# snowflakezzz/FAST-LIVO-noted

Measured on AMD Instinct MI355X. Metric: IEKF scan-to-map updates/sec (100k-pt scan, 1M-pt map), higher is better.
Workload: dtype f32+f64; 1 GPU; config2: 100k-pt scan vs 1M-pt map, max_iteration=4, 8 independent scans per GPU per step; scan_points=100000, map_points=1000000, parallelism=scan farm x1

## Files before the change

fast-livo-noted_amd/csrc/livo_capi.cpp:

```cpp
#include <hip/hip_runtime.h>

#include <algorithm>
#include <cmath>
#include <cstdio>
#include <cstdlib>
#include <cstring>
#include <new>
#include <chrono>
#include <thread>
#include <vector>

#include "carve.h"
#include "livo_internal.h"

using namespace livo;

namespace {

struct ScanBuf {
    bool used = false;
    int64_t n = 0;
    int32_t nblk = 0;
    float* pts = nullptr;
    NNRec* nn = nullptr;
// ... 138 lines not shown
    int32_t dvlog2 = 4;
    int64_t d_n = 0, dslot_cap = 0, dpts_cap = 0;
    int64_t rebases = 0;
    double rebase_frac = 0.125;
    float min_gh = 0.f;
    float max_gh = 0.f;
    float box_cell = 1.2f;
    float box_cell_max = 2.0f;
    float* gpts_alt = nullptr;
    int64_t gpts_alt_cap = 0;
    int64_t grid_ids = -1, cells = -1;
    float grid_gh = 0.f;
    bool merge = true;
    int64_t rebuilds_sorted = 0, rebuilds_merged = 0;
    int64_t wide_redos = 0;
    int64_t rebuilds_fused = 0;
    ScanCtx scan;
};

struct Staging {
    char* h = nullptr;
    char* d = nullptr;
    char* h_dev = nullptr;
    size_t cap = 0;
    void free() {
        if (d) (void)hipFree(d);
        if (h) (void)hipHostFree(h);
        h = d = h_dev = nullptr;
        cap = 0;
    }
    int ensure(size_t bytes) {
        if (bytes <= cap) return LIVO_OK;
        free();
        if (hipMalloc((void**)&d, bytes) != hipSuccess) {
            d = nullptr;
            return LIVO_E_OOM;
        }
        if (hipHostMalloc((void**)&h, bytes, hipHostMallocMapped | hipHostMallocCoherent) != hipSuccess) {
            h = nullptr;
            return LIVO_E_OOM;
        }
        if (hipHostGetDevicePointer((void**)&h_dev, h, 0) != hipSuccess) {
            (void)hipGetLastError();
            h_dev = nullptr;
        }
        cap = bytes;
        return LIVO_OK;
    }
};

struct BatchPlan {
    int model = 0;
    int32_t n = 0;
    bool fused = false;
    bool kcopy = false;
    bool wb = false;
    bool iv = false;
    bool lazy = false;
    int prof = 0;
    Staging* stage = nullptr;
    size_t stride = 0;
    int ngroups = 0;
    struct Group {
        int32_t first, count;
        int max_nblk;
        int64_t max_n, off;
        hipStream_t st;
    } g[kMaxGroups];
};

struct BatchLane {
    Staging stage[2];
    hipStream_t st[kMaxGroups] = {};
    hipEvent_t done[kMaxGroups] = {};
    bool busy = false;
    int32_t ticket = -1;
    int32_t n = 0;
    BatchPlan plan;
    std::vector<int32_t> ids;
};

constexpr int kPinRing = 16;

struct livo_ctx {
    int device = 0;
    hipStream_t stream = nullptr;
    hipStream_t xstream[kMaxGroups - 1] = {};
    hipEvent_t xjoin[kMaxGroups - 1] = {};
    int groups = 0;
    int leaf_size = kLeafSize;
    livo_params params{};
    MapNode* nodes = nullptr;
    int64_t map_points = 0;
    int64_t map_slots = 0;
    int32_t map_depth = 0;
    LeafNode* lnodes = nullptr;
    float* lpts = nullptr;
    int32_t leaf_depth = 0;
    int64_t leaf_bytes = 0;
    int knn_kind = 2;
// ... 37 lines not shown
    DevImage match_img;
    void* vm_buf = nullptr;
    size_t vm_bytes = 0;
    void* prim_tmp = nullptr;
    size_t prim_bytes = 0;
    std::vector<ScanBuf> scans;
    std::vector<ScanBuf> spare;
    void* up_tmp = nullptr;
    size_t up_tmp_bytes = 0;
    hipStream_t up_stream = nullptr;
    void* aup_tmp = nullptr;
    size_t aup_tmp_bytes = 0;
    void* aup_prim = nullptr;
    size_t aup_prim_bytes = 0;
    struct PinSlot {
        float* h = nullptr;
        size_t bytes = 0;
        hipEvent_t copied = nullptr;
        bool inflight = false;
    } pin[kPinRing];
    int pin_next = 0;
    hipStream_t cp_stream = nullptr;
    void* bsrc[2] = {nullptr, nullptr};
    size_t bsrc_bytes[2] = {0, 0};
    hipEvent_t bsrc_copied[2] = {nullptr, nullptr};
    hipEvent_t bsrc_free[2] = {nullptr, nullptr};
    bool bsrc_used[2] = {false, false};
    int bsrc_next = 0;
    IekfSlot* d_slots = nullptr;
    BatchLane lane[LIVO_MAX_INFLIGHT];
    int32_t lane_gen = 0;
    bool lane_serial = false;
    bool slot_wb = true;
    bool rec_compact = true;
    bool rec_lazy = true;
    bool eval_gen = false;
    int last_lane = -1;
    unsigned long long last_replays = 0;
    IekfSlot* h_slots = nullptr;
    HsJob* d_jobs = nullptr;
    HsJob* h_jobs = nullptr;
    unsigned* d_replay_count = nullptr;
    unsigned long long* d_replay_total = nullptr;
    unsigned long long* d_replay_list = nullptr;
    int64_t replay_cap = 0;
    unsigned* d_replay_count2 = nullptr;
    unsigned long long* d_replay_list2 = nullptr;
    void* scratch = nullptr;
    size_t scratch_bytes = 0;
    void* rec_tmp = nullptr;
    size_t rec_tmp_bytes = 0;
    int profiling = 0;
    hipEvent_t ev[kMaxGroups][3 * LIVO_MAX_EVALS + 2] = {};
    hipEvent_t b_start = nullptr, b_end[2] = {};
    int b_par = 0;
    bool b_prev = false;
    bool events_ready = false;
    livo_timings last{};
};

#define HIP_TRY(x)                                  \
    do {                                            \
        if ((x) != hipSuccess) return LIVO_E_HIP;   \
    } while (0)
#define RC_TRY(x)                  \
    do {                           \
// ... 1318 lines not shown
    livo_params def;
    livo_params_default(&def);
    if (p && !params_valid(p)) return LIVO_E_INVALID;
    int ndev = 0;
    if (hipGetDeviceCount(&ndev) != hipSuccess || ndev <= 0) return LIVO_E_HIP;
    if (device < 0 || device >= ndev) return LIVO_E_INVALID;
    livo_ctx* c = new (std::nothrow) livo_ctx();
    if (!c) return LIVO_E_OOM;
    c->device = device;
    c->params = p ? *p : def;
    if (const char* env = std::getenv("LIVO_STREAM_GROUPS")) {
        const int v = std::atoi(env);
        if (v >= 1 && v <= kMaxGroups) c->groups = v;
    }
    if (const char* env = std::getenv("LIVO_LEAF_SIZE")) {
        const int v = std::atoi(env);
        if (v >= 2 && v <= 256) c->leaf_size = v;
    }
    if (const char* env = std::getenv("LIVO_FUSED")) c->fused = std::atoi(env) != 0;
    if (const char* env = std::getenv("LIVO_KNN_KIND"))
        c->knn_kind = std::strcmp(env, "leaf") == 0 ? 0 : std::strcmp(env, "grid") == 0 ? 1 : 2;
    if (const char* env = std::getenv("LIVO_VRUNS")) c->vruns = std::atoi(env) != 0;
    if (const char* env = std::getenv("LIVO_BRUNS")) c->bruns = std::atoi(env) != 0;
    if (const char* env = std::getenv("LIVO_BR_HA")) {
        const float v = (float)std::atof(env);
        if (v > 0.2f && v < 20.f) c->br_ha = v;
    }
    if (const char* env = std::getenv("LIVO_BR_R")) {
        const float v = (float)std::atof(env);
        if (v > 0.5f && v < 20.f) c->br_r = v;
    }
    if (const char* env = std::getenv("LIVO_LANE_SERIAL")) c->lane_serial = std::atoi(env) != 0;
    if (const char* env = std::getenv("LIVO_SLOT_WB")) c->slot_wb = std::atoi(env) != 0;
    if (const char* env = std::getenv("LIVO_REC_COMPACT")) c->rec_compact = std::atoi(env) != 0;
    if (const char* env = std::getenv("LIVO_REC_LAZY")) c->rec_lazy = std::atoi(env) != 0;
    if (const char* env = std::getenv("LIVO_EVAL_GEN")) c->eval_gen = std::atoi(env) != 0;
    if (const char* env = std::getenv("LIVO_XCD_CHUNK")) c->xcd_chunk = std::max(0, std::atoi(env));
    if (const char* env = std::getenv("LIVO_GRID_PPC")) {
        const float v = (float)std::atof(env);
        if (v > 0.f) c->grid_ppc = v;
    }
    if (const char* env = std::getenv("LIVO_GRID_CELL")) {
        const float v = (float)std::atof(env);
        if (v > 0.f) c->grid_cell = v;
    }
    if (set_device(c) || hipStreamCreateWithFlags(&c->stream, hipStreamNonBlocking) != hipSuccess ||
        create_group_streams(c)) {
        delete c;
        return LIVO_E_HIP;
    }
    *out = c;
    return LIVO_OK;
}

int livo_ctx_destroy(livo_ctx* c) {
    if (!c) return LIVO_E_INVALID;
    (void)hipSetDevice(c->device);
    if (c->stream) (void)hipStreamSynchronize(c->stream);
    for (int k = 0; k < kMaxGroups - 1; k++)
        if (c->xstream[k]) (void)hipStreamSynchronize(c->xstream[k]);
    if (c->up_stream) (void)hipStreamSynchronize(c->up_stream);
    if (c->cp_stream) (void)hipStreamSynchronize(c->cp_stream);
    for (int k = 0; k < 2; k++) {
        if (c->bsrc[k]) (void)hipFree(c->bsrc[k]);
        if (c->bsrc_copied[k]) (void)hipEventDestroy(c->bsrc_copied[k]);
        if (c->bsrc_free[k]) (void)hipEventDestroy(c->bsrc_free[k]);
// ... 1257 lines not shown
    std::sort(sorted.begin(), sorted.end());
    if (std::adjacent_find(sorted.begin(), sorted.end()) != sorted.end()) return LIVO_E_INVALID;
    for (int l = 0; l < LIVO_MAX_INFLIGHT; l++)
        if (l != L && c->lane[l].busy)
            for (int32_t id : c->lane[l].ids)
                if (std::binary_search(sorted.begin(), sorted.end(), id)) return LIVO_E_INVALID;
    if (!batch_fused(c, model) && model != kModelIkfom && (L != 0 || !sync)) return LIVO_E_INVALID;
    return LIVO_OK;
}

static int64_t batch_plan(livo_ctx* c, int L, int32_t n, const int32_t* ids, int model, bool sync) {
    BatchLane& B = c->lane[L];
    BatchPlan& P = B.plan;
    P.model = model;
    P.n = n;
    P.fused = batch_fused(c, model);
    P.stage = &B.stage[model];
    P.stride = model == kModelIkfom ? sizeof(IekfSlot) : kLmStride;
    P.kcopy = !sync && P.stage->h_dev;
    P.wb = P.fused && P.stage->h_dev && c->slot_wb;
    P.iv = c->backend == LIVO_BACKEND_IVOX && model != kModelIkfom;
    P.prof = sync && L == 0 && c->events_ready ? c->profiling : 0;
    const int auto_groups = (P.fused || model == kModelIkfom) ? 4 : 2;
    P.ngroups = std::max(1, std::min<int>(c->groups > 0 ? c->groups : auto_groups, n));
    int64_t off = 0;
    for (int gi = 0; gi < P.ngroups; gi++) {
        BatchPlan::Group& G = P.g[gi];
        G.first = (int32_t)((int64_t)n * gi / P.ngroups);
        G.count = (int32_t)((int64_t)n * (gi + 1) / P.ngroups) - G.first;
        G.max_nblk = 1;
        G.max_n = 1;
        G.off = off;
        G.st = B.st[gi];
        for (int32_t b = G.first; b < G.first + G.count; b++) {
            const ScanBuf* s = get_scan_q(c, ids[b]);
            G.max_nblk = std::max(G.max_nblk, (int)s->nblk);
            G.max_n = std::max<int64_t>(G.max_n, s->n);
            off += s->n;
        }
    }
    return off;
}

static void batch_fill(livo_ctx* c, const BatchPlan& P, const int32_t* ids, const livo_state* states,
                       const livo_state* priors, const livo_ikfom_state* ik_states) {
    HsJob* const hjobs = reinterpret_cast<HsJob*>(P.stage->h + (size_t)P.n * P.stride);
    const int max_iter = c->params.max_iterations;
    for (int32_t b = 0; b < P.n; b++) {
        if (P.model == kModelIkfom) {
            init_slot_ik(hslot(P, b), ik_states[b], max_iter);
        } else {
            init_slot(hslot(P, b), states[b], priors ? priors[b] : states[b], max_iter, kSlotLmBytes);
        }
        fill_job(hjobs[b], *get_scan_q(c, ids[b]), dslot(P, b));
        if (P.wb) hjobs[b].host_slot = reinterpret_cast<uint4*>(P.stage->h_dev + (size_t)b * P.stride);
    }
}

static unsigned* lane_rcount(livo_ctx* c, int L) { return c->d_replay_count + (size_t)L * kMaxGroups; }

static int stage_group(livo_ctx* c, int L, const BatchPlan& P, int gi, const int32_t* ids, const BatchLane* prev) {
    static_assert(sizeof(HsJob) % 16 == 0 && sizeof(IekfSlot) % 16 == 0 && kLmStride % 16 == 0, "16-B word copies");
    const BatchPlan::Group& G = P.g[gi];
    const hipStream_t st = G.st;
    for (int32_t b = G.first; b < G.first + G.count; b++) {
        ScanBuf* s = get_scan_q(c, ids[b]);
        if (s->pending) HIP_TRY(hipStreamWaitEvent(st, s->ready, 0));
        if (P.model == kModelIkfom && s->n > 0) HIP_TRY(hipMemsetAsync(s->pstate, 0, (size_t)s->n, st));
        if (!P.fused) RC_TRY(ensure_nn_coords(c, s, st));
    }
    if (prev)
        for (int q = 0; q < prev->plan.ngroups; q++) HIP_TRY(hipStreamWaitEvent(st, prev->done[q], 0));
    const size_t s0 = (size_t)G.first * P.stride, sb = (size_t)G.count * P.stride;
    const size_t j0 = (size_t)P.n * P.stride + (size_t)G.first * sizeof(HsJob), jb = (size_t)G.count * sizeof(HsJob);
    if (P.kcopy) {
        RC_TRY(launch_copy_ranges(P.stage->h_dev, P.stage->d, s0, sb, j0, jb, st));
    } else {
        HIP_TRY(hipMemcpyAsync(P.stage->d + s0, P.stage->h + s0, sb, hipMemcpyHostToDevice, st));
        HIP_TRY(hipMemcpyAsync(P.stage->d + j0, P.stage->h + j0, jb, hipMemcpyHostToDevice, st));
    }
    if (!P.fused) HIP_TRY(hipMemsetAsync(lane_rcount(c, L) + gi, 0, sizeof(unsigned), st));
    if (P.iv) HIP_TRY(hipMemsetAsync(c->d_replay_count2 + gi, 0, sizeof(unsigned), st));
    HIP_TRY(prof_record(P, kProfAny, c->ev[gi][0], st));
    return LIVO_OK;
}

static void group_params(livo_ctx* c, int L, const BatchPlan& P, int gi, KnnParams& kp, HsParams& hp) {
    const BatchPlan::Group& G = P.g[gi];
    HsJob* const jobs = reinterpret_cast<HsJob*>(P.stage->d + (size_t)P.n * P.stride) + G.first;
    hp = make_hs_params(c);
    hp.jobs = jobs;
    kp = make_knn_params(c);
    kp.jobs = jobs;
    kp.replay_count = lane_rcount(c, L) + gi;
    kp.replay_list = c->d_replay_list + (size_t)L * c->replay_cap + G.off;
    kp.replay_count2 = P.iv ? c->d_replay_count2 + gi : nullptr;
    kp.replay_list2 = P.iv ? c->d_replay_list2 + G.off : nullptr;
    if (kp.iv.scratch) kp.iv.scratch += (int64_t)gi * c->iv.big_threads * c->iv.big_slice;
    hp.solve = P.model == kModelIkfom ? 0 : 1;
    hp.replay_count = kp.replay_count;
    hp.replay_count2 = kp.replay_count2;
}

static int queue_fused(livo_ctx* c, const BatchPlan& P, const int32_t* ids, const KnnParams* kp, const HsParams* hp) {
    for (int32_t b = 0; b < P.n; b++) {
        ScanBuf* s = get_scan_q(c, ids[b]);
        s->nn_lazy = false;
        if (kp[0].rec_compact) s->nn_compact = true;
    }
    const int evals = c->params.max_iterations + 1;
    for (int e = 0; e < evals; e++)
        for (int gi = 0; gi < P.ngroups; gi++) {
            const BatchPlan::Group& G = P.g[gi];
            if (e > 0) HIP_TRY(prof_record(P, kProfL2, c->ev[gi][e], G.st));
            RC_TRY(launch_iekf_eval(kp[gi], hp[gi], G.count, G.max_n, e == 0, G.st));
            if (e == 0) HIP_TRY(prof_record(P, kProfL1, c->ev[gi][1], G.st));
        }
    return LIVO_OK;
}

static int queue_unfused(livo_ctx* c, const BatchPlan& P, const KnnParams* kp, const HsParams* hp) {
    const int evals = c->params.max_iterations + 1;
    const bool ik = P.model == kModelIkfom;
    for (int e = 0; e < evals; e++)
        for (int gi = 0; gi < P.ngroups; gi++) {
            const BatchPlan::Group& G = P.g[gi];
            if (e > 0) HIP_TRY(prof_record(P, kProfL2, c->ev[gi][3 * e], G.st));
            RC_TRY(backend_knn(c, kp[gi], G.count, G.max_n, e > 0, G.st));
            HIP_TRY(prof_record(P, e == 0 ? kProfAny : kProfL2, c->ev[gi][3 * e + 1], G.st));
            RC_TRY(ik ? launch_hshare_ik(hp[gi], G.count, G.max_nblk, e == 0, G.st)
                      : launch_hshare(hp[gi], G.count, G.max_nblk, e == 0, G.st));
            if (ik) RC_TRY(launch_solve_ik(hp[gi], G.count, G.st));
        }
    return LIVO_OK;
}

static int finish_group(livo_ctx* c, BatchLane& B, const BatchPlan& P, int gi) {
    const BatchPlan::Group& G = P.g[gi];
    const int last_ev = P.fused ? c->params.max_iterations + 1 : 3 * LIVO_MAX_EVALS;
    HIP_TRY(prof_record(P, kProfL2, c->ev[gi][last_ev], G.st));
    if (P.wb) {
    } else if (P.kcopy) {
        RC_TRY(launch_copy_words(dslot(P, G.first), P.stage->h_dev + (size_t)G.first * P.stride, P.stride * G.count,
                                 G.st));
    } else {
        HIP_TRY(hipMemcpyAsync(&hslot(P, G.first), dslot(P, G.first), P.stride * G.count, hipMemcpyDeviceToHost, G.st));
    }
    HIP_TRY(hipEventRecord(B.done[gi], G.st));
// ... 1449 lines not shown
```

fast-livo-noted_amd/csrc/livo_internal.h:

```cpp
#pragma once
#include <math.h>
#include <stddef.h>
#include <stdint.h>

#include "cam_model.h"
#include "vmap_model.h"
#include "livo.h"
#include "stl_select.h"

#ifndef LIVO_PTS_PER_THREAD
#define LIVO_PTS_PER_THREAD 1
#endif

namespace livo {

constexpr int kRunPad = 8;

constexpr int kNN = LIVO_NUM_MATCH_POINTS;
constexpr int kDim = LIVO_DIM_STATE;
constexpr int kBlock = 256;
#ifndef LIVO_KNN_BLOCK
#define LIVO_KNN_BLOCK 128
#endif
constexpr int kKnnBlock = LIVO_KNN_BLOCK;
// ... 282 lines not shown
    int32_t rec_lazy;
    int32_t eval_gen;
};

struct SolveParams {
    IekfSlot* slots;
    const HsJob* jobs;
    unsigned* replay_count;
    int32_t mode;
};

struct HostMap {
    MapNode* nodes = nullptr;
    int64_t num_points = 0;
    int64_t num_slots = 0;
    int32_t depth = 0;
};
int build_host_map(const float* xyz, int64_t M, int64_t stride_bytes, HostMap* out);
void free_host_map(HostMap* m);

size_t knn_lds_bytes(int depth);
int launch_knn_pass(const KnnParams& p, int n_jobs, int64_t max_n, void* stream);
int launch_knn_leaf(const KnnParams& p, int n_jobs, int64_t max_n, bool seeded, void* stream);
int launch_knn_grid(const KnnParams& p, int n_jobs, int64_t max_n, bool seeded, bool tile, void* stream);
int launch_hshare(const HsParams& p, int n_jobs, int max_nblk, bool first, void* stream);
#ifndef LIVO_EVAL_BLOCK
#define LIVO_EVAL_BLOCK 256
#endif
constexpr int kEvalBlock = LIVO_EVAL_BLOCK;
enum EvalKind : int { kEvalRunsStatic = 0, kEvalGeneric = 1 };
#ifndef LIVO_EVAL_WAVES
#define LIVO_EVAL_WAVES 5
#endif
int launch_iekf_eval(const KnnParams& kp, const HsParams& hp, int n_jobs, int64_t max_n, bool first, void* stream);
int launch_solve_ik(const HsParams& p, int n_jobs, void* stream);
int launch_copy_words(const void* src, void* dst, size_t bytes, void* stream);
int launch_copy_ranges(const void* src, void* dst, size_t o0, size_t n0, size_t o1, size_t n1, void* stream);
int launch_hshare_ik(const HsParams& p, int n_jobs, int max_nblk, bool first, void* stream);
int launch_solve(const SolveParams& p, int n_jobs, void* stream);

int launch_ivox_clear(GridSlot* slots, int64_t table, void* stream);
int launch_ivox_insert(const IvoxParams& p, void* stream);
int launch_ivox_rollback(const IvoxParams& p, void* stream);
int launch_ivox_prepare(const IvoxParams& p, void* stream);
int launch_ivox_move(const IvoxParams& p, void* stream);
int launch_ivox_place(const IvoxParams& p, void* stream);
int launch_ivox_fix(const IvoxParams& p, void* stream);
int launch_ivox_rehash(const GridSlot* old_slots, const unsigned long long* old_t, int64_t old_table, GridSlot* slots,
                       unsigned long long* tlast, int log2, void* stream);
int launch_ivox_newfirst(const IvoxParams& p, uint32_t* out, unsigned long long* n, void* stream);
int launch_ivox_oldkeys(const IvoxParams& p, unsigned long long* keys, uint32_t* slot, unsigned long long* n,
                        void* stream);
int launch_ivox_untouched(const IvoxParams& p, const uint32_t* sorted_slot, int64_t n, uint32_t* flags, void* stream);
int launch_ivox_oldfirst(const IvoxParams& p, const uint32_t* sorted_slot, int64_t n, uint32_t* out, void* stream);
int launch_ivox_victims(const IvoxParams& p, const uint32_t* sorted_slot, const uint32_t* rank, int64_t n, int64_t ev,
                        uint32_t j_first, void* stream);
int launch_ivox_tcur_min(const IvoxParams& p, void* stream);
int launch_ivox_mark_min(const IvoxParams& p, void* stream);
int launch_ivox_drop(const IvoxParams& p, void* stream);
int launch_ivox_commit(const IvoxParams& p, void* stream);
int launch_ivox_knn(const KnnParams& p, int n_jobs, int64_t max_n, bool later, int64_t overflow_threads,
                    void* stream);
int prim_sort_pairs_u32(void* temp, size_t* temp_bytes, const uint32_t* keys_in, uint32_t* keys_out,
                        const uint32_t* vals_in, uint32_t* vals_out, int64_t n, int bits, void* stream);
int prim_exclusive_scan_u32(void* temp, size_t* temp_bytes, const uint32_t* in, uint32_t* out, int64_t n,
                            void* stream);
struct MapIncrParams {
// ... 347 lines not shown
```

fast-livo-noted_amd/csrc/livo_kernels.hip:

```cpp
#include <hip/hip_runtime.h>
#include <math.h>

#include <utility>

#include "livo_internal.h"
#include "device_common.h"
#include "device_linalg.h"

#if defined(LIVO_EVAL_PROF) && !defined(LIVO_TAIL_PROF)
#define LIVO_TAIL_PROF
#endif

namespace livo {

template <class T>
__device__ __forceinline__ const __attribute__((address_space(1))) T* gptr(const T* p) {
    return (const __attribute__((address_space(1))) T*)p;
}
template <class T>
__device__ __forceinline__ __attribute__((address_space(1))) T* gptr(T* p) {
    return (__attribute__((address_space(1))) T*)p;
}
constexpr double kMtkTol = 1e-11;
constexpr double kS2Len = 98090.0 / 10000.0;
// ... 2296 lines not shown
    bfly_stage<0x1B>(x, 4, (l & 2) == 0);
    bfly_stage<0xB1>(x, 2, (l & 1) == 0);
    const int base = ((l & 8) ? 16 : 0) + ((l & 4) ? 8 : 0) + ((l & 2) ? 4 : 0) + ((l & 1) ? 2 : 0);
    if (base < NU) R.red[(tid >> 4) * kRedCols + base] = x[0];
    if (base + 1 < NU) R.red[(tid >> 4) * kRedCols + base + 1] = x[1];
}

#ifdef LIVO_TAIL_PROF
__device__ unsigned long long g_tail_prof[3][8];
#define TAIL_MARK(k, t)                                                                                 \
    do {                                                                                               \
        if (pk >= 0 && threadIdx.x == 0) {                                                             \
            const unsigned long long now_ = __builtin_amdgcn_s_memtime();                             \
            atomicAdd(&g_tail_prof[pk][(k)], now_ - (t));                                              \
            (t) = now_;                                                                                \
        }                                                                                              \
    } while (0)
#else
#define TAIL_MARK(k, t) do { } while (0)
#endif
#ifndef LIVO_RED_INFLIGHT
#define LIVO_RED_INFLIGHT 32
#endif
constexpr int kRedInFlight = LIVO_RED_INFLIGHT;
__device__ __forceinline__ void hs_host_slot(const HsJob& job, const IekfSlot* slot, int t, int nt) {
    const unsigned long long* src = reinterpret_cast<const unsigned long long*>(slot);
    for (int w = t; w < (int)((kSlotWbBytes + 15) / 16); w += nt) {
        const unsigned long long lo = __hip_atomic_load(gptr(src + 2 * w), __ATOMIC_RELAXED, __HIP_MEMORY_SCOPE_AGENT);
        const unsigned long long hi = __hip_atomic_load(gptr(src + 2 * w + 1), __ATOMIC_RELAXED, __HIP_MEMORY_SCOPE_AGENT);
        job.host_slot[w] = make_uint4((unsigned)lo, (unsigned)(lo >> 32), (unsigned)hi, (unsigned)(hi >> 32));
    }
}

template <int NT, int NU, class Col>
__device__ __forceinline__ void hs_block_partial(const HsJob& job, const Col& col, unsigned blk, HsReduceLds& R) {
    const int tid = threadIdx.x;
    constexpr int NR = NT / 16;
    static_assert(NR <= kRedRows, "HsReduceLds row partials");
    constexpr int NRM = NR > 16 ? NR : 16;
    hs_row_sums_bfly<NU>(col, R, tid, std::make_integer_sequence<int, 32>{});
    __syncthreads();
    if (tid < NU) {
        double r[NRM];
#pragma unroll
        for (int w = 0; w < NRM; w++) r[w] = w < NR ? R.red[w * kRedCols + tid] : 0.0;
#pragma unroll
        for (int h = NRM / 2; h >= 1; h >>= 1)
#pragma unroll
            for (int w = 0; w < h; w++) r[w] = r[w] + r[w + h];
        const double v = r[0];
        __hip_atomic_store(gptr(job.partial + (size_t)blk * kRedCols + tid), v, __ATOMIC_RELAXED, __HIP_MEMORY_SCOPE_AGENT);
    }
}

template <int NT, int NU>
__device__ __forceinline__ void hs_scan_tail(const HsParams& P, const HsJob& job, IekfSlot* slot, int nblk,
                                             HsReduceLds& R, SolveLds& L, int pk
#ifdef LIVO_TAIL_PROF
                                             , unsigned long long tp
#endif
);

template <int NT, int NU = kRedUsed>
__device__ __forceinline__ bool hs_shard_level(const HsJob& job, IekfSlot* slot, int nblk, unsigned blk,
                                               HsReduceLds& R) {
    static_assert(NU == kRedUsed || NU == kRedUsed + 2, "h_share sums (+ search counts)");
    static_assert(NT / 32 <= kRedRows / 2, "R.fin holds one row per 32-thread group");
    const int tid = threadIdx.x;
    const int K = nblk < kRedShards ? nblk : kRedShards;
    const int sh = (int)(blk % (unsigned)K);
    const int cnt = (nblk - sh + K - 1) / K;
    unsigned* const sh_ticket = slot->sh_ticket + 32 * sh;
    if (tid < 64) {
        asm volatile("s_waitcnt vmcnt(0)" ::: "memory");
        if (tid == 0)
            R.last = __hip_atomic_fetch_add(gptr(sh_ticket), 1u, __ATOMIC_RELAXED, __HIP_MEMORY_SCOPE_AGENT) ==
                     (unsigned)cnt - 1u;
    }
    __syncthreads();
    if (!R.last) return false;
    if (cnt > 1) {
        constexpr int G = NT / 32;
        constexpr int kMaxPer = 8;
        const int c = tid & 31, g = tid >> 5;
        double acc = 0.0;
        if (c < NU) {
            const double* src = job.partial + c;
            for (int j0 = g; j0 < cnt; j0 += kMaxPer * G) {
                double v[kMaxPer];
#pragma unroll
                for (int k = 0; k < kMaxPer; k++) {
                    const int j = j0 + G * k;
                    v[k] = j < cnt ? ld_sc1(src + (size_t)(sh + K * j) * kRedCols) : 0.0;
                }
#pragma unroll
                for (int k = 0; k < kMaxPer; k++) acc += v[k];
            }
        }
        R.fin[g * kRedCols + c] = acc;
        __syncthreads();
        if (tid < NU) {
            constexpr int NG = G > 8 ? G : 8;
            double f[NG];
#pragma unroll
            for (int q = 0; q < NG; q++) f[q] = q < G ? R.fin[q * kRedCols + tid] : 0.0;
#pragma unroll
            for (int h = NG / 2; h >= 1; h >>= 1)
#pragma unroll
                for (int q = 0; q < h; q++) f[q] = f[2 * q] + f[2 * q + 1];
            st_sc1(job.partial + (size_t)sh * kRedCols + tid, f[0]);
        }
    }
    if (tid < 64) {
        if (tid == 0) st_sc1(sh_ticket, 0u);
        asm volatile("s_waitcnt vmcnt(0)" ::: "memory");
    }
    return true;
}

template <int NT, int NU = kRedUsed>
__device__ __forceinline__ void hs_ticket_tail(const HsParams& P, const HsJob& job, IekfSlot* slot, int nblk,
                                               unsigned blk, HsReduceLds& R, SolveLds& L, int pk = -1) {
    const int tid = threadIdx.x;
#ifdef LIVO_TAIL_PROF
    unsigned long long tp = __builtin_amdgcn_s_memtime();
    if (pk >= 0 && tid == 0) atomicAdd(&g_tail_prof[pk][0], 1ull);
#else
    (void)pk;
#endif
    if (!hs_shard_level<NT, NU>(job, slot, nblk, blk, R)) return;
    TAIL_MARK(1, tp);
    const int K = nblk < kRedShards ? nblk : kRedShards;
    if (tid == 0)
        R.last2 = __hip_atomic_fetch_add(gptr(&slot->hs_ticket), 1u, __ATOMIC_RELAXED, __HIP_MEMORY_SCOPE_AGENT) ==
                  (unsigned)K - 1u;
    __syncthreads();
    if (!R.last2) return;
#ifdef LIVO_TAIL_PROF
    hs_scan_tail<NT, NU>(P, job, slot, K, R, L, pk, tp);
#else
    hs_scan_tail<NT, NU>(P, job, slot, K, R, L, pk);
#endif
}

template <int NT, int NU>
__device__ __forceinline__ void hs_scan_tail(const HsParams& P, const HsJob& job, IekfSlot* slot, int nblk,
                                             HsReduceLds& R, SolveLds& L, int pk
#ifdef LIVO_TAIL_PROF
                                             , unsigned long long tp
#endif
) {
    const int tid = threadIdx.x;
    __builtin_amdgcn_s_setprio(3);
#ifdef LIVO_TAIL_PROF
    if (pk >= 0 && tid == 0) atomicAdd(&g_tail_prof[pk][5], 1ull);
#endif
    const bool solve = P.solve != 0;
    if (solve) solve_stage(slot, L, tid, NT);
    {
        constexpr int G = NT / 32;
        const int c = tid & 31, g = tid >> 5;
        double acc = 0.0;
        if (c < NU) {
            double* src = job.partial + c;
            for (int b0 = g; b0 < nblk; b0 += kRedInFlight * G) {
                double v[kRedInFlight];
#pragma unroll
                for (int k = 0; k < kRedInFlight; k++) {
                    const int b = b0 + G * k;
                    v[k] = b < nblk ? ld_sc1(src + (size_t)b * kRedCols) : 0.0;
                }
#pragma unroll
                for (int k = 0; k < kRedInFlight; k++) acc += v[k];
            }
        }
        R.fin[g * kRedCols + c] = acc;
    }
    __syncthreads();
    const bool wb = solve && job.host_slot != nullptr;
    if (tid >= 64) {
        if (solve && tid == 64) state_minus_d(L.pr, L.st, L.vec);
        if (solve) __syncthreads();
        if (wb) {
            __syncthreads();
            if (L.ctrl.stop) hs_host_slot(job, slot, tid, NT);
        }
        return;
    }
    TAIL_MARK(2, tp);
    if (tid < kRedCols) {
        double v = 0.0;
        if (tid < NU) {
            constexpr int NG = NT / 32 > 8 ? NT / 32 : 8;
            double f[NG];
#pragma unroll
            for (int g = 0; g < NG; g++) f[g] = g < NT / 32 ? R.fin[g * kRedCols + tid] : 0.0;
#pragma unroll
            for (int h = NG / 2; h >= 1; h >>= 1)
#pragma unroll
                for (int g = 0; g < h; g++) f[g] = f[2 * g] + f[2 * g + 1];
            v = f[0];
        }
        if (NU > kRedUsed && tid >= kRedUsed) {
            if (tid < NU && v > 0.0) {
                int e = solve ? L.ctrl.n_evals : slot->ctrl.n_evals;
                e = e < LIVO_MAX_EVALS ? e : LIVO_MAX_EVALS - 1;
                atomicAdd((tid == kRedUsed ? slot->visits : slot->scanned) + e, (unsigned long long)v);
            }
            v = 0.0;
        }
        L.sum[tid] = v;
        slot->red[tid] = v;
    }
    if (tid == 0) st_sc1(&slot->hs_ticket, 0u);
    if (!solve) return;
    WAVE_SYNC();
    solve_scan<true>(slot, L, tid, pk);
    TAIL_MARK(3, tp);
    if (wb) {
        asm volatile("s_waitcnt vmcnt(0)" ::: "memory");
        __syncthreads();
        if (L.ctrl.stop) hs_host_slot(job, slot, tid, NT);
    }
#ifdef LIVO_TAIL_PROF
    asm volatile("s_waitcnt vmcnt(0)" ::: "memory");
#endif
    TAIL_MARK(4, tp);
}

template <int NT, int NU = kRedUsed, class Col>
__device__ __forceinline__ void hshare_reduce_solve(const HsParams& P, const HsJob& job, IekfSlot* slot,
                                                    const Col& col, int nblk, unsigned blk, HsReduceLds& R,
                                                    SolveLds& L, int pk = -1) {
    hs_block_partial<NT, NU>(job, col, blk, R);
    hs_ticket_tail<NT, NU>(P, job, slot, nblk, blk, R, L, pk);
}

template <bool FIRST>
__global__ __launch_bounds__(kBlock) void k_hshare(HsParams P) {
    __shared__ HsReduceLds R;
    __shared__ SolveLds L;
    const HsJob job = P.jobs[blockIdx.y];
    if (P.replay_count && blockIdx.x == 0 && blockIdx.y == 0 && threadIdx.x == 0) *P.replay_count = 0u;
    if (P.replay_count2 && blockIdx.x == 0 && blockIdx.y == 0 && threadIdx.x == 0) *P.replay_count2 = 0u;
    if ((int)blockIdx.x >= job.nblk) return;
    IekfSlot* slot = job.slot;
    int search;
    if (P.force >= 0) {
        search = P.force;
    } else {
        if (slot->ctrl.stop) return;
        search = FIRST ? 1 : slot->ctrl.search_en;
    }
    const livo_state& S = slot->state;
    double acc[kRedUsed];
#pragma unroll
    for (int j = 0; j < kRedUsed; j++) acc[j] = 0.0;
    for (int rep = 0; rep < kPtsPerThread; rep++) {
        const int i = (blockIdx.x * kPtsPerThread + rep) * kBlock + threadIdx.x;
        if (i < job.n) {
            HsRow w;
            hs_row_clear(w);
            HsPointIn in = hshare_load(job, i, !search);
            hshare_point(P, job, S, i, search, w, in);
            hs_accumulate(acc, w, P.inv_r);
        }
    }
    hshare_reduce_solve<kBlock>(P, job, slot, [&](auto jc) { return acc[decltype(jc)::value]; }, job.nblk,
                                blockIdx.x, R, L);
}

#ifndef LIVO_EVAL_TILE_CELLS
#define LIVO_EVAL_TILE_CELLS 256
#endif
#ifndef LIVO_EVAL_TILE_PTS
#define LIVO_EVAL_TILE_PTS 1024
#endif
using BlockTile = TileLds<LIVO_EVAL_TILE_CELLS, LIVO_EVAL_TILE_PTS>;

__device__ __forceinline__ void replay_wave(const KnnParams& P, const HsJob& job, int i, bool amb, float4* cache,
                                            const PoseRef& pose) {
    unsigned long long m = __ballot(amb);
    const int lane = (int)(threadIdx.x & 63u);
    while (m) {
        const int l = __ffsll((long long)m) - 1;
        m &= m - 1ull;
        const int il = __shfl(i, l);
        float qx, qy, qz;
        query_point(P, pose, reinterpret_cast<const float4*>(job.pts)[il], qx, qy, qz);
        Cands c;
        knn_exact_wave(P.nodes, P.n_nodes, P.has_map, qx, qy, qz, cache, c);
        if (lane == l) {
            float od[kNN];
            uint32_t on[kNN];
#pragma unroll
            for (int k = 0; k < kNN; k++) { od[k] = c.d[k]; on[k] = c.node[k]; }
            write_nnrec(job.nn + il, P.nodes, c.n, od, on, rec_flag(job.nn[il].cf) | 0x100);
        }
    }
}

struct EvalParams {
    KnnParams k;
    HsParams h;
};

#ifdef LIVO_EVAL_PROF
__device__ unsigned long long g_eval_prof[3][8];
__device__ unsigned long long g_eval_stats[3][8];
#define EVAL_MARK(k)                                                                                   \
    do {                                                                                               \
        if (threadIdx.x == 0) {                                                                        \
            const unsigned long long now = __builtin_amdgcn_s_memtime();                              \
            if ((k) > 0) atomicAdd(&g_eval_prof[FIRST ? 2 : (search ? 1 : 0)][(k)], now - prof_t);     \
            else atomicAdd(&g_eval_prof[FIRST ? 2 : (search ? 1 : 0)][0], 1ull);       \
            prof_t = now;                                                                              \
        }                                                                                              \
    } while (0)
#define EVAL_MARK_SYNC(k) do { __syncthreads(); EVAL_MARK(k); } while (0)
constexpr int kTlBlocks = 4096;
__device__ unsigned long long g_eval_tl[LIVO_MAX_EVALS][kTlBlocks][2];
#define EVAL_PROF_DECL unsigned long long prof_t = 0
#else
#define EVAL_MARK(k) do { } while (0)
#define EVAL_MARK_SYNC(k) do { } while (0)
#define EVAL_PROF_DECL do { } while (0)
#endif
struct EvalRsLds {
    HsReduceLds R;
    SolveLds solve;
};
template <int KIND>
union EvalLds {
    BlockTile tile;
    EvalRsLds rs;
    float4 nnstage[kEvalBlock / 64][64 * 4];
};
template <>
union EvalLds<kEvalRunsStatic> {
    EvalRsLds rs;
    float4 nnstage[kEvalBlock / 64][64 * 4];
};
template <bool FIRST, int KIND>
__device__ __forceinline__ void iekf_eval_body(const EvalParams& E, EvalLds<KIND>& U) {
    constexpr bool kStatic = KIND == kEvalRunsStatic;
    const KnnParams& P = E.k;
    EVAL_PROF_DECL;
#ifdef LIVO_EVAL_PROF
    const unsigned long long tl_start = __builtin_amdgcn_s_memtime();
#endif
    unsigned bjob, bx;
    xcd_chunk_block(P.nb, P.xcd_chunk, bjob, bx);
    const HsJob job = P.jobs[bjob];
    IekfSlot* slot = job.slot;
    if (bx > 0 && (int)bx * kEvalBlock >= job.n) return;
    const int i = (int)bx * kEvalBlock + threadIdx.x;
    const bool valid = i < job.n;
    HsPointIn pin = !FIRST && valid ? hshare_load(job, i, true) : HsPointIn{};
    bool prefit = false;
    if (slot->ctrl.stop) return;
    const int search = FIRST ? 1 : slot->ctrl.search_en;
    bool dead = false;
#ifndef LIVO_EVAL_PROF
    if constexpr (kStatic) {
        const IekfCtrl& c = slot->ctrl;
        dead = P.rec_compact && E.h.solve && !E.h.dbg.normvec && !E.h.dbg.world && !E.h.dbg.sel;
        if constexpr (FIRST)
            dead = dead && c.max_iter >= 2 && c.max_iter + 1 <= LIVO_MAX_EVALS && c.iter_count == -1 &&
                   c.rematch_num == 0 && c.n_evals == 0;
        else
            dead = dead && P.rec_lazy;
    }
#endif
    const PoseRef pose{slot->state.rot, slot->state.pos};
#ifdef LIVO_EVAL_PROF
    const int tl_e = min(slot->ctrl.n_evals, LIVO_MAX_EVALS - 1);
#endif
    EVAL_MARK(0);
    unsigned n_slots = 0u, n_pts = 0u;
    if (search) {
        pin = HsPointIn{};
        LeafQuery q;
        lq_init<false>(q, P, pose, job, i, valid);
        int c0 = 0, c1 = 0, c2 = 0, s0 = 1, s1 = 1, s2 = 1;
        if (valid) grid_cell(P, q, c0, c1, c2, s0, s1, s2);
        unsigned visits = 0, npts = 0;
        bool amb = false;
        const bool canon = !kStatic && P.canon;
        if (kStatic || P.vslots) {
            EVAL_MARK(1);
            bool certified = false;
#ifdef LIVO_EVAL_PROF
            const unsigned np0 = npts;
            bool ball_ok = false;
#endif
            const bool dyn = !kStatic && P.dyn_runs != 0;
            if (P.bslots) {
                certified = dyn ? brun_search<true>(q, P, valid, visits, npts) : brun_search<false>(q, P, valid, visits, npts);
                if (valid && !certified) lq_init<false>(q, P, pose, job, i, valid);
#ifdef LIVO_EVAL_PROF
                ball_ok = certified;
#endif
            }
#ifdef LIVO_EVAL_PROF
            const unsigned np1 = npts;
#endif
            if (!certified)
                certified = dyn ? vrun_search<true>(q, P, valid, c0, c1, c2, s0, s1, s2, visits, npts)
                                : vrun_search<false>(q, P, valid, c0, c1, c2, s0, s1, s2, visits, npts);
// ... 108 lines not shown
        if (valid) pin.pb = reinterpret_cast<const float4*>(job.pts)[i];
        if (amb) atomicAdd(P.replay_total, 1ull);
        if (canon) {
            if (amb) canon_query(P, job, i, pose);
            __syncthreads();
        } else if (__syncthreads_or(amb)) {
            static_assert(sizeof(U) >= (size_t)(kEvalBlock / 64) * (4u << kReplayLevels) * sizeof(float4),
                          "replay caches do not fit the evaluation's LDS");
            float4* cache = reinterpret_cast<float4*>(&U) + (threadIdx.x >> 6) * (4u << kReplayLevels);
            replay_wave(P, job, i, amb, cache, pose);
            __syncthreads();
        }
        EVAL_MARK(2);
    }
    HsRow w;
    hs_row_clear(w);
    const int nblk = max(1, (job.n + kEvalBlock - 1) / kEvalBlock);
    if (valid) {
        hshare_point(E.h, job, pose, i, search, w, pin, prefit);
    }
    EVAL_MARK_SYNC(3);
    const double inv_r = E.h.inv_r;
    auto col = [&](auto jc) -> double {
        constexpr int j = decltype(jc)::value;
        if constexpr (j < kRedUsed) return hs_col<j>(w, inv_r);
        else if constexpr (j == kRedUsed) return (double)n_slots;
        else return (double)n_pts;
    };
#ifdef LIVO_TAIL_PROF
    const int pk = FIRST ? 2 : (search ? 1 : 0);
#else
    const int pk = -1;
#endif
    hshare_reduce_solve<kEvalBlock, kRedUsed + 2>(E.h, job, slot, col, nblk, bx, U.rs.R, U.rs.solve, pk);
    EVAL_MARK(4);
#ifdef LIVO_EVAL_PROF
    if (threadIdx.x == 0 && blockIdx.x < (unsigned)kTlBlocks) {
        g_eval_tl[tl_e][blockIdx.x][0] = tl_start;
        g_eval_tl[tl_e][blockIdx.x][1] = __builtin_amdgcn_s_memtime();
    }
#endif
}
template <bool FIRST>
__global__ __launch_bounds__(kEvalBlock, LIVO_EVAL_WAVES) void k_iekf_eval(EvalParams E) {
    __shared__ EvalLds<kEvalRunsStatic> U;
    iekf_eval_body<FIRST, kEvalRunsStatic>(E, U);
}
template <bool FIRST>
__global__ __launch_bounds__(kEvalBlock, 4) void k_iekf_eval_gen(EvalParams E) {
    __shared__ EvalLds<kEvalGeneric> U;
    iekf_eval_body<FIRST, kEvalGeneric>(E, U);
}

constexpr int kIkDrop = 0x1000;

struct IkSolveLds {
    double P[kIkDim * kIkDim];
    double Pinv[kIkDim * kIkDim];
    double LU[kIkDim * kIkDim];
    double L[kIkDim * kIkDim];
    double Kx[kIkDim * 12];
    double sum[kIkCols];
    double dx[kIkDim], dxn[kIkDim], dxu[kIkDim], Kh[kIkDim];
    double J[9];
    double Hm[kIkFewRows * 13];
    double Km[kIkDim * kIkFewRows];
    int piv[kIkDim];
// ... 648 lines not shown
    for (int64_t i = (int64_t)blockIdx.x * 256 + threadIdx.x; i < n16; i += (int64_t)gridDim.x * 256) dst[i] = src[i];
}

int launch_copy_words(const void* src, void* dst, size_t bytes, void* stream) {
    if (bytes == 0) return LIVO_OK;
    if (bytes % 16 || (reinterpret_cast<uintptr_t>(src) | reinterpret_cast<uintptr_t>(dst)) % 16) return LIVO_E_INVALID;
    const int64_t n16 = (int64_t)(bytes / 16);
    const unsigned blocks = (unsigned)std::min<int64_t>((n16 + 255) / 256, 64);
    hipLaunchKernelGGL(k_copy_words, dim3(blocks), dim3(256), 0, (hipStream_t)stream,
                       reinterpret_cast<const uint4*>(src), reinterpret_cast<uint4*>(dst), n16);
    return hipGetLastError() == hipSuccess ? LIVO_OK : LIVO_E_HIP;
}

__global__ __launch_bounds__(256) void k_copy_ranges(const uint4* __restrict__ src, uint4* __restrict__ dst,
                                                     int64_t a0, int64_t n0, int64_t a1, int64_t n1) {
    for (int64_t i = (int64_t)blockIdx.x * 256 + threadIdx.x; i < n0 + n1; i += (int64_t)gridDim.x * 256) {
        const int64_t w = i < n0 ? a0 + i : a1 + (i - n0);
        dst[w] = src[w];
    }
}

int launch_copy_ranges(const void* src, void* dst, size_t o0, size_t n0, size_t o1, size_t n1, void* stream) {
    if (n0 + n1 == 0) return LIVO_OK;
    if ((o0 | n0 | o1 | n1) % 16 || (reinterpret_cast<uintptr_t>(src) | reinterpret_cast<uintptr_t>(dst)) % 16)
        return LIVO_E_INVALID;
    const int64_t w0 = (int64_t)(n0 / 16), w1 = (int64_t)(n1 / 16);
    const unsigned blocks = (unsigned)std::min<int64_t>((w0 + w1 + 255) / 256, 64);
    hipLaunchKernelGGL(k_copy_ranges, dim3(blocks), dim3(256), 0, (hipStream_t)stream,
                       reinterpret_cast<const uint4*>(src), reinterpret_cast<uint4*>(dst), (int64_t)(o0 / 16), w0,
                       (int64_t)(o1 / 16), w1);
    return hipGetLastError() == hipSuccess ? LIVO_OK : LIVO_E_HIP;
}

int launch_iekf_eval(const KnnParams& kp, const HsParams& hp, int n_jobs, int64_t max_n, bool first, void* stream) {
    if (n_jobs <= 0 || max_n <= 0) return LIVO_OK;
    EvalParams E;
    E.k = kp;
    E.h = hp;
    E.k.nb = (int32_t)((max_n + kEvalBlock - 1) / kEvalBlock);
    if ((int64_t)E.k.nb * n_jobs >= (1ll << 31)) return LIVO_E_RANGE;
    const dim3 grid((unsigned)(E.k.nb * n_jobs)), block(kEvalBlock);
    const bool stat = kp.vslots && !kp.dyn_runs && !kp.canon && !kp.eval_gen;
    if (stat) {
        if (first)
            hipLaunchKernelGGL(k_iekf_eval<true>, grid, block, 0, (hipStream_t)stream, E);
        else
            hipLaunchKernelGGL(k_iekf_eval<false>, grid, block, 0, (hipStream_t)stream, E);
    } else {
        if (first)
            hipLaunchKernelGGL(k_iekf_eval_gen<true>, grid, block, 0, (hipStream_t)stream, E);
        else
            hipLaunchKernelGGL(k_iekf_eval_gen<false>, grid, block, 0, (hipStream_t)stream, E);
    }
    return hipGetLastError() == hipSuccess ? LIVO_OK : LIVO_E_HIP;
}

int launch_hshare(const HsParams& p, int n_jobs, int max_nblk, bool first, void* stream) {
    if (n_jobs <= 0 || max_nblk <= 0) return LIVO_OK;
    dim3 grid(max_nblk, n_jobs), block(kBlock);
    if (first)
        hipLaunchKernelGGL(k_hshare<true>, grid, block, 0, (hipStream_t)stream, p);
    else
        hipLaunchKernelGGL(k_hshare<false>, grid, block, 0, (hipStream_t)stream, p);
    return hipGetLastError() == hipSuccess ? LIVO_OK : LIVO_E_HIP;
}

int launch_hshare_ik(const HsParams& p, int n_jobs, int max_nblk, bool first, void* stream) {
    if (n_jobs <= 0 || max_nblk <= 0) return LIVO_OK;
    dim3 grid(max_nblk, n_jobs), block(kBlock);
    if (first)
        hipLaunchKernelGGL(k_hshare_ik<true>, grid, block, 0, (hipStream_t)stream, p);
// ... 21 lines not shown
```

Baseline: 34520 scan updates/s.

## Pass job descriptors and initial pose inline via kernel arguments, skip staging copy

When a group holds few scans and zero-copy write-back is enabled, job records and the initial pose/ctrl head are embedded in the eval kernel's argument block. The per-group host-to-device staging copy kernel is then skipped. On the first eval the tail solver reads the slot straight from mapped host memory and writes it through to the device slot. This removes one copy launch and its dependency from each batch's critical path. The cost is a larger kernarg block, extra uncached host reads in the first tail, and a hipMemset plus device sync when the staging buffer grows.

```diff
diff --git a/fast-livo-noted_amd/csrc/livo_capi.cpp b/fast-livo-noted_amd/csrc/livo_capi.cpp
--- a/fast-livo-noted_amd/csrc/livo_capi.cpp
+++ b/fast-livo-noted_amd/csrc/livo_capi.cpp
@@ -194,7 +194,10 @@
     int ensure(size_t bytes) {
         if (bytes <= cap) return LIVO_OK;
         free();
-        if (hipMalloc((void**)&d, bytes) != hipSuccess) {
+        if (hipMalloc((void**)&d, bytes) != hipSuccess || hipMemset(d, 0, bytes) != hipSuccess ||
+            hipDeviceSynchronize() != hipSuccess) {
+            (void)hipGetLastError();
+            if (d) (void)hipFree(d);
             d = nullptr;
             return LIVO_E_OOM;
         }
@@ -228,6 +231,7 @@
         int max_nblk;
         int64_t max_n, off;
         hipStream_t st;
+        bool inl;
     } g[kMaxGroups];
 };
 
@@ -331,6 +335,7 @@
     int32_t lane_gen = 0;
     bool lane_serial = false;
     bool slot_wb = true;
+    bool stage_copy = false;
     bool rec_compact = true;
     bool rec_lazy = true;
     bool eval_gen = false;
@@ -1715,6 +1720,7 @@
     }
     if (const char* env = std::getenv("LIVO_LANE_SERIAL")) c->lane_serial = std::atoi(env) != 0;
     if (const char* env = std::getenv("LIVO_SLOT_WB")) c->slot_wb = std::atoi(env) != 0;
+    if (const char* env = std::getenv("LIVO_STAGE_COPY")) c->stage_copy = std::atoi(env) != 0;
     if (const char* env = std::getenv("LIVO_REC_COMPACT")) c->rec_compact = std::atoi(env) != 0;
     if (const char* env = std::getenv("LIVO_REC_LAZY")) c->rec_lazy = std::atoi(env) != 0;
     if (const char* env = std::getenv("LIVO_EVAL_GEN")) c->eval_gen = std::atoi(env) != 0;
@@ -3038,6 +3044,7 @@
         G.max_n = 1;
         G.off = off;
         G.st = B.st[gi];
+        G.inl = P.fused && P.kcopy && P.wb && !c->stage_copy && G.count <= kInlineJobs;
         for (int32_t b = G.first; b < G.first + G.count; b++) {
             const ScanBuf* s = get_scan_q(c, ids[b]);
             G.max_nblk = std::max(G.max_nblk, (int)s->nblk);
@@ -3079,7 +3086,8 @@
         for (int q = 0; q < prev->plan.ngroups; q++) HIP_TRY(hipStreamWaitEvent(st, prev->done[q], 0));
     const size_t s0 = (size_t)G.first * P.stride, sb = (size_t)G.count * P.stride;
     const size_t j0 = (size_t)P.n * P.stride + (size_t)G.first * sizeof(HsJob), jb = (size_t)G.count * sizeof(HsJob);
-    if (P.kcopy) {
+    if (G.inl) {
+    } else if (P.kcopy) {
         RC_TRY(launch_copy_ranges(P.stage->h_dev, P.stage->d, s0, sb, j0, jb, st));
     } else {
         HIP_TRY(hipMemcpyAsync(P.stage->d + s0, P.stage->h + s0, sb, hipMemcpyHostToDevice, st));
@@ -3115,11 +3123,28 @@
         if (kp[0].rec_compact) s->nn_compact = true;
     }
     const int evals = c->params.max_iterations + 1;
+    EvalInline inl[kMaxGroups];
+    const HsJob* const hjobs = reinterpret_cast<const HsJob*>(P.stage->h + (size_t)P.n * P.stride);
+    for (int gi = 0; gi < P.ngroups; gi++) {
+        const BatchPlan::Group& G = P.g[gi];
+        if (!G.inl) continue;
+        EvalInline& I = inl[gi];
+        std::memset(&I, 0, sizeof(I));
+        I.n = G.count;
+        for (int32_t k = 0; k < G.count; k++) {
+            const IekfSlot& s = hslot(P, G.first + k);
+            I.jobs[k] = hjobs[G.first + k];
+            std::memcpy(I.head[k].rot, s.state.rot, sizeof(I.head[k].rot));
+            std::memcpy(I.head[k].pos, s.state.pos, sizeof(I.head[k].pos));
+            I.head[k].ctrl = s.ctrl;
+        }
+    }
     for (int e = 0; e < evals; e++)
         for (int gi = 0; gi < P.ngroups; gi++) {
             const BatchPlan::Group& G = P.g[gi];
             if (e > 0) HIP_TRY(prof_record(P, kProfL2, c->ev[gi][e], G.st));
-            RC_TRY(launch_iekf_eval(kp[gi], hp[gi], G.count, G.max_n, e == 0, G.st));
+            if (G.inl) inl[gi].first_in = e == 0;
+            RC_TRY(launch_iekf_eval(kp[gi], hp[gi], G.count, G.max_n, e == 0, G.st, G.inl ? &inl[gi] : nullptr));
             if (e == 0) HIP_TRY(prof_record(P, kProfL1, c->ev[gi][1], G.st));
         }
     return LIVO_OK;
diff --git a/fast-livo-noted_amd/csrc/livo_internal.h b/fast-livo-noted_amd/csrc/livo_internal.h
--- a/fast-livo-noted_amd/csrc/livo_internal.h
+++ b/fast-livo-noted_amd/csrc/livo_internal.h
@@ -338,7 +338,27 @@
 #ifndef LIVO_EVAL_WAVES
 #define LIVO_EVAL_WAVES 5
 #endif
-int launch_iekf_eval(const KnnParams& kp, const HsParams& hp, int n_jobs, int64_t max_n, bool first, void* stream);
+constexpr int kInlineJobs = 4;
+struct alignas(16) EvalHead {
+    double rot[9], pos[3];
+    IekfCtrl ctrl;
+};
+static_assert(sizeof(EvalHead) == 128, "128 B a scan");
+struct EvalInline {
+    int32_t n;
+    int32_t first_in;
+    int32_t pad_[2];
+    HsJob jobs[kInlineJobs];
+    EvalHead head[kInlineJobs];
+};
+struct EvalParams {
+    KnnParams k;
+    HsParams h;
+    EvalInline in;
+};
+static_assert(sizeof(EvalParams) <= 4096, "kernel arguments: one 4-KB segment");
+int launch_iekf_eval(const KnnParams& kp, const HsParams& hp, int n_jobs, int64_t max_n, bool first, void* stream,
+                     const EvalInline* inl = nullptr);
 int launch_solve_ik(const HsParams& p, int n_jobs, void* stream);
 int launch_copy_words(const void* src, void* dst, size_t bytes, void* stream);
 int launch_copy_ranges(const void* src, void* dst, size_t o0, size_t n0, size_t o1, size_t n1, void* stream);
diff --git a/fast-livo-noted_amd/csrc/livo_kernels.hip b/fast-livo-noted_amd/csrc/livo_kernels.hip
--- a/fast-livo-noted_amd/csrc/livo_kernels.hip
+++ b/fast-livo-noted_amd/csrc/livo_kernels.hip
@@ -2352,6 +2352,27 @@
     }
 }
 
+constexpr int kSlotThroughWords = (int)(offsetof(IekfSlot, sh_ticket) / 8);
+static_assert(offsetof(IekfSlot, sh_ticket) % 8 == 0 && offsetof(IekfSlot, sh_ticket) + sizeof(IekfSlot::sh_ticket) == kSlotLmBytes,
+              "the shard tickets end the LaserMapping slot");
+template <int NT>
+__device__ __forceinline__ void slot_through_t(const IekfSlot* src, IekfSlot* slot, int t) {
+    constexpr int kPer = (kSlotThroughWords + NT - 1) / NT;
+    const unsigned long long* s = reinterpret_cast<const unsigned long long*>(src);
+    unsigned long long* d = reinterpret_cast<unsigned long long*>(slot);
+    unsigned long long v[kPer];
+#pragma unroll
+    for (int k = 0; k < kPer; k++) {
+        const int w = t + k * NT;
+        v[k] = w < kSlotThroughWords ? ld_sc1(s + w) : 0ull;
+    }
+#pragma unroll
+    for (int k = 0; k < kPer; k++) {
+        const int w = t + k * NT;
+        if (w < kSlotThroughWords) st_sc1(d + w, v[k]);
+    }
+}
+
 template <int NT, int NU, class Col>
 __device__ __forceinline__ void hs_block_partial(const HsJob& job, const Col& col, unsigned blk, HsReduceLds& R) {
     const int tid = threadIdx.x;
@@ -2379,7 +2400,7 @@
 #ifdef LIVO_TAIL_PROF
                                              , unsigned long long tp
 #endif
-);
+                                             , bool first_in = false);
 
 template <int NT, int NU = kRedUsed>
 __device__ __forceinline__ bool hs_shard_level(const HsJob& job, IekfSlot* slot, int nblk, unsigned blk,
@@ -2440,7 +2461,8 @@
 
 template <int NT, int NU = kRedUsed>
 __device__ __forceinline__ void hs_ticket_tail(const HsParams& P, const HsJob& job, IekfSlot* slot, int nblk,
-                                               unsigned blk, HsReduceLds& R, SolveLds& L, int pk = -1) {
+                                               unsigned blk, HsReduceLds& R, SolveLds& L, int pk = -1,
+                                               bool first_in = false) {
     const int tid = threadIdx.x;
 #ifdef LIVO_TAIL_PROF
     unsigned long long tp = __builtin_amdgcn_s_memtime();
@@ -2457,9 +2479,9 @@
     __syncthreads();
     if (!R.last2) return;
 #ifdef LIVO_TAIL_PROF
-    hs_scan_tail<NT, NU>(P, job, slot, K, R, L, pk, tp);
+    hs_scan_tail<NT, NU>(P, job, slot, K, R, L, pk, tp, first_in);
 #else
-    hs_scan_tail<NT, NU>(P, job, slot, K, R, L, pk);
+    hs_scan_tail<NT, NU>(P, job, slot, K, R, L, pk, first_in);
 #endif
 }
 
@@ -2469,14 +2491,16 @@
 #ifdef LIVO_TAIL_PROF
                                              , unsigned long long tp
 #endif
-) {
+                                             , bool first_in) {
     const int tid = threadIdx.x;
     __builtin_amdgcn_s_setprio(3);
 #ifdef LIVO_TAIL_PROF
     if (pk >= 0 && tid == 0) atomicAdd(&g_tail_prof[pk][5], 1ull);
 #endif
     const bool solve = P.solve != 0;
-    if (solve) solve_stage(slot, L, tid, NT);
+    const IekfSlot* const stage_in = first_in ? reinterpret_cast<const IekfSlot*>(job.host_slot) : nullptr;
+    if (solve) solve_stage(stage_in ? stage_in : slot, L, tid, NT);
+    if (stage_in) slot_through_t<NT>(stage_in, slot, tid);
     {
         constexpr int G = NT / 32;
         const int c = tid & 31, g = tid >> 5;
@@ -2496,6 +2520,7 @@
         }
         R.fin[g * kRedCols + c] = acc;
     }
+    if (stage_in) asm volatile("s_waitcnt vmcnt(0)" ::: "memory");
     __syncthreads();
     const bool wb = solve && job.host_slot != nullptr;
     if (tid >= 64) {
@@ -2551,9 +2576,9 @@
 template <int NT, int NU = kRedUsed, class Col>
 __device__ __forceinline__ void hshare_reduce_solve(const HsParams& P, const HsJob& job, IekfSlot* slot,
                                                     const Col& col, int nblk, unsigned blk, HsReduceLds& R,
-                                                    SolveLds& L, int pk = -1) {
+                                                    SolveLds& L, int pk = -1, bool first_in = false) {
     hs_block_partial<NT, NU>(job, col, blk, R);
-    hs_ticket_tail<NT, NU>(P, job, slot, nblk, blk, R, L, pk);
+    hs_ticket_tail<NT, NU>(P, job, slot, nblk, blk, R, L, pk, first_in);
 }
 
 template <bool FIRST>
@@ -2619,11 +2644,6 @@
         }
     }
 }
-
-struct EvalParams {
-    KnnParams k;
-    HsParams h;
-};
 
 #ifdef LIVO_EVAL_PROF
 __device__ unsigned long long g_eval_prof[3][8];
@@ -2671,19 +2691,36 @@
 #endif
     unsigned bjob, bx;
     xcd_chunk_block(P.nb, P.xcd_chunk, bjob, bx);
-    const HsJob job = P.jobs[bjob];
+    using CWord = const __attribute__((address_space(4))) unsigned long long;
+    HsJob job;
+    {
+        constexpr int kW = (int)(sizeof(HsJob) / 8);
+        static_assert(sizeof(HsJob) % 8 == 0, "HsJob in 8-B words");
+        CWord* const src = E.in.n > 0 ? (CWord*)&E.in.jobs[bjob] : (CWord*)&P.jobs[bjob];
+        unsigned long long w[kW];
+#pragma unroll
+        for (int k = 0; k < kW; k++) w[k] = src[k];
+        __builtin_memcpy(&job, w, sizeof(HsJob));
+    }
     IekfSlot* slot = job.slot;
+    const bool first_in = FIRST && E.in.first_in != 0;
+    const EvalHead& head = *reinterpret_cast<const EvalHead*>(
+        (const char*)__builtin_amdgcn_kernarg_segment_ptr() + offsetof(EvalParams, in.head) +
+        (first_in ? bjob : 0u) * sizeof(EvalHead));
+    IekfCtrl ctrl_in;
+    if (first_in) ctrl_in = head.ctrl;
+    else ctrl_in = slot->ctrl;
     if (bx > 0 && (int)bx * kEvalBlock >= job.n) return;
     const int i = (int)bx * kEvalBlock + threadIdx.x;
     const bool valid = i < job.n;
     HsPointIn pin = !FIRST && valid ? hshare_load(job, i, true) : HsPointIn{};
     bool prefit = false;
-    if (slot->ctrl.stop) return;
+    if (ctrl_in.stop) return;
     const int search = FIRST ? 1 : slot->ctrl.search_en;
     bool dead = false;
 #ifndef LIVO_EVAL_PROF
     if constexpr (kStatic) {
-        const IekfCtrl& c = slot->ctrl;
+        const IekfCtrl& c = ctrl_in;
         dead = P.rec_compact && E.h.solve && !E.h.dbg.normvec && !E.h.dbg.world && !E.h.dbg.sel;
         if constexpr (FIRST)
             dead = dead && c.max_iter >= 2 && c.max_iter + 1 <= LIVO_MAX_EVALS && c.iter_count == -1 &&
@@ -2692,9 +2729,12 @@
             dead = dead && P.rec_lazy;
     }
 #endif
-    const PoseRef pose{slot->state.rot, slot->state.pos};
+    static_assert(offsetof(livo_state, pos) == 9 * sizeof(double) && offsetof(EvalHead, pos) == 9 * sizeof(double) &&
+                      offsetof(IekfSlot, state) == 0 && offsetof(livo_state, rot) == 0, "pose: rot[9], pos[3]");
+    const double* const pose_b = first_in ? head.rot : slot->state.rot;
+    const PoseRef pose{pose_b, pose_b + 9};
 #ifdef LIVO_EVAL_PROF
-    const int tl_e = min(slot->ctrl.n_evals, LIVO_MAX_EVALS - 1);
+    const int tl_e = min(ctrl_in.n_evals, LIVO_MAX_EVALS - 1);
 #endif
     EVAL_MARK(0);
     unsigned n_slots = 0u, n_pts = 0u;
@@ -2869,7 +2909,8 @@
 #else
     const int pk = -1;
 #endif
-    hshare_reduce_solve<kEvalBlock, kRedUsed + 2>(E.h, job, slot, col, nblk, bx, U.rs.R, U.rs.solve, pk);
+    hshare_reduce_solve<kEvalBlock, kRedUsed + 2>(E.h, job, slot, col, nblk, bx, U.rs.R, U.rs.solve, pk,
+                                                  FIRST && E.in.first_in != 0);
     EVAL_MARK(4);
 #ifdef LIVO_EVAL_PROF
     if (threadIdx.x == 0 && blockIdx.x < (unsigned)kTlBlocks) {
@@ -3584,11 +3625,16 @@
     return hipGetLastError() == hipSuccess ? LIVO_OK : LIVO_E_HIP;
 }
 
-int launch_iekf_eval(const KnnParams& kp, const HsParams& hp, int n_jobs, int64_t max_n, bool first, void* stream) {
+int launch_iekf_eval(const KnnParams& kp, const HsParams& hp, int n_jobs, int64_t max_n, bool first, void* stream,
+                     const EvalInline* inl) {
     if (n_jobs <= 0 || max_n <= 0) return LIVO_OK;
+    if (inl && (inl->n != n_jobs || n_jobs > kInlineJobs || (inl->first_in && !first))) return LIVO_E_INVALID;
+    for (int k = 0; inl && k < n_jobs; k++)
+        if (!inl->jobs[k].host_slot) return LIVO_E_INVALID;
     EvalParams E;
     E.k = kp;
     E.h = hp;
+    E.in = inl ? *inl : EvalInline{};
     E.k.nb = (int32_t)((max_n + kEvalBlock - 1) / kEvalBlock);
     if ((int64_t)E.k.nb * n_jobs >= (1ll << 31)) return LIVO_E_RANGE;
     const dim3 grid((unsigned)(E.k.nb * n_jobs)), block(kEvalBlock);
```

New measurement: 36000 scan updates/s, median of 6. 1.04x the previous value.
